# hpsim/OGL

Measured on AMD Instinct MI355X. Metric: cg_iters_per_sec, higher is better.
Workload: dtype f64

## Files before the change

### ogl_amd/csrc/kernels.hpp

```cpp
#pragma once
#include <hip/hip_runtime.h>

#include "common.hpp"

namespace ogl {

struct DevCriterion {
    double tolerance, rel_tol;
    int32_t min_iter, max_iter, frequency, export_res;
};

struct DevScalars {
    double rho, prev_rho, beta;
    double alpha, omega, gamma;
    double norm_factor;
    double init_res, res;
    double xbar;
    double sums[4];
    int32_t iter;
    int32_t stop;
    int32_t n_evals;
    int32_t stop_phase;
    int32_t stop_turn;
    int32_t comm_error;
// ... 63 lines not shown
    const int32_t *chunk_bptr = nullptr;
    const int32_t *boundary_rows = nullptr;
    const int32_t *entry_ptrs = nullptr;
    const int32_t *cols = nullptr;
    const double *vals = nullptr;
    const double *recv = nullptr;
    const unsigned long long *local_flag = nullptr;
    int32_t n_neigh = 0;
    uint32_t seq = 0;
    long long timeout_ticks = 0;
    DevScalars *s = nullptr;
};
void launch_spmv(hipStream_t st, const DevCsr &A, int mode, const double *x, const double *b,
                 double *y, const SpmvDots &dots, const DevScalars *gate, const HaloFused &hf = HaloFused{});

struct DevEll {
    int32_t n_rows = 0;
    int32_t width = 0;
    int64_t stride = 0;
    const int32_t *cols = nullptr;
    const double *vals = nullptr;
    bool stream = false;
};
void launch_spmv_ell(hipStream_t st, const DevEll &A, int mode, const double *x, const double *b,
                     double *y, const SpmvDots &dots, const DevScalars *gate, const HaloFused &hf = HaloFused{});
struct DevSell {
    int32_t n_rows = 0;
    const SellChunk *chunks = nullptr;
    const int32_t *dict = nullptr;
    const uint8_t *codes = nullptr;
    const double *vals = nullptr;
    const int32_t *spill_chunk_ptr = nullptr, *spill_rows = nullptr, *spill_ptrs = nullptr, *spill_cols = nullptr;
    const double *spill_vals = nullptr;
    bool stream = false;
    int32_t xcd_group = 0;
    const uint16_t *rmap = nullptr;
    const int32_t *block_order = nullptr;
    int32_t n_blocks = 0;
};
void launch_spmv_sell(hipStream_t st, const DevSell &A, int mode, const double *x, const double *b,
                      double *y, const SpmvDots &dots, const DevScalars *gate, const HaloFused &hf = HaloFused{});
struct DevSym {
    int32_t n_rows = 0;
    int32_t nd = 0;
    int32_t d[4] = {0, 0, 0, 0};
    const uint8_t *mask = nullptr;
    const double *planes = nullptr;
    bool stream = false;
    const int32_t *block_order = nullptr;
    int32_t n_blocks = 0;
};
void launch_spmv_sym(hipStream_t st, const DevSym &A, int mode, const double *x, const double *b, double *y,
                     const SpmvDots &dots, const DevScalars *gate, const HaloFused &hf = HaloFused{});
struct DevSymx {
    int32_t n_rows = 0;
    const SymxChunk *chunks = nullptr, *chunks_general = nullptr;
    int32_t n_blocks_general = 0;
    const uint8_t *mask = nullptr;
    const double *planes = nullptr;
    const int32_t *ex_rowptr = nullptr, *ex_cols = nullptr;
    const int32_t *ex_lrow = nullptr;
    const double *ex_vals = nullptr;
    bool stream = false;
    bool fast = false;
    int32_t xcd_group = 0;
    int32_t n_blocks = 0;
};
void launch_spmv_symx(hipStream_t st, const DevSymx &A, int mode, const double *x, const double *b, double *y,
                      const SpmvDots &dots, const DevScalars *gate, const HaloFused &hf = HaloFused{});
void launch_gather_coeffs_masked(hipStream_t st, int64_t n, const int32_t *map, const double *source,
                                 double *out);
void launch_gather_sell(hipStream_t st, int32_t n_chunks, const SellChunk *chunks, const int32_t *map,
                        const double *source, double *out);

void launch_spmv_non_local(hipStream_t st, const DevHalo &H, int mode, const double *recv,
                           double *y, const DevScalars *gate);
void launch_pack(hipStream_t st, const DevHalo &H, const double *x, double *send,
                 const DevScalars *gate);

void launch_gather_coeffs(hipStream_t st, int32_t nnz, const int32_t *ldu_mapping,
                          const double *source, double *coeffs);
void launch_jacobi_generate(hipStream_t st, const DevCsr &A, double *inv_diag);
void launch_jacobi_generate_pos(hipStream_t st, const DevCsr &A, const int32_t *diag_pos, double *inv_diag);
void launch_jacobi_generate_diag(hipStream_t st, int32_t n_rows, const double *diag, double *inv_diag);

struct DevBlockJacobi {
    int32_t n_rows = 0;
    int32_t n_blocks = 0;
    int32_t stride = 0;
    const int32_t *block_ptrs = nullptr;
    const int32_t *row_block = nullptr;
    double *blocks = nullptr;
    int32_t uniform = 0;
    const int32_t *rows = nullptr, *pos = nullptr;
    int32_t by_device_row = 0;
    int32_t perm_xcd_group = 0;
};
constexpr int MAX_JACOBI_BLOCK = 32;
void launch_bj_generate(hipStream_t st, const DevCsr &A, const DevBlockJacobi &J,
                        bool group_lanes = true);
void launch_bj_apply(hipStream_t st, const DevBlockJacobi &J, const double *in, double *out,
                     double *dot_part, const DevScalars *gate);
void launch_bj_apply_staged(hipStream_t st, const DevBlockJacobi &J, const double *in, double *out, double *dot_part,
                            const DevScalars *gate, double *tmp_in, double *tmp_out);

constexpr int ISAI_THREAD_ROW = 32;
// ... 336 lines not shown
```

### ogl_amd/csrc/kernels_krylov.hip

```cpp
#include "device_common.hpp"
#include "resident_cg_turn.hpp"

namespace ogl {

namespace {

__global__ __launch_bounds__(BLOCK) void k_scale(int n, double *__restrict__ v, double f)
{
    const int i = blockIdx.x * BLOCK + threadIdx.x;
    if (i < n) v[i] = v[i] * f;
}

__global__ __launch_bounds__(BLOCK) void k_fill_xbar(int n, double *__restrict__ v,
                                                     const DevScalars *s)
{
    const int i = blockIdx.x * BLOCK + threadIdx.x;
    if (i < n) v[i] = s->xbar;
}

enum PartialOp { P_SUM = 0, P_DOT = 1, P_NORM1 = 2 };
template <int OP>
__global__ __launch_bounds__(BLOCK) void k_partials(int n, int n_chunks,
                                                    const double *__restrict__ a,
                                                    const double *__restrict__ b,
// ... 238 lines not shown
        part_norm[chunk] = s1;
    }
    if (PUT) {
        __shared__ double ps[CHUNK_ROWS];
        __shared__ int last;
        halo_put_chunk(put, chunk, vz.x, vz.y, ps, &last);
    }
}


template <bool LEAD, int K>
__global__ __launch_bounds__(BLOCK) void k_cg_step1x_fin(int n, double *p, double *__restrict__ x,
                                                         const double *__restrict__ r,
                                                         const double *__restrict__ inv_diag,
                                                         const DevScalars *sin, DevScalars *sout,
                                                         const double *__restrict__ part_rho,
                                                         const double *__restrict__ part_norm, int n_part,
                                                         double *history, int first, LeadBox lead,
                                                         double *p_out, PRing ring)
{
    __shared__ double red[2 * FIN_WAVES];
    __shared__ double sh[4];
    __shared__ int sh_stop;
    __shared__ double lead_words[LEAD ? LEAD_BOX_WORDS / 2 : 1];
    __shared__ double lead_stage[LEAD ? LEAD_STAGE : 1];
    __shared__ int lead_timed_out;
    const uint32_t seq = LEAD ? sin->launch_seq : 0u;
    if (LEAD) lead_leaders<2>(lead, seq, part_rho, part_norm, nullptr, n_part, lead_stage);
    const int stopped = sin->stop;
    const double s_rho = sin->rho, s_beta = sin->beta, s_nf = sin->norm_factor, s_init = sin->init_res;
    const int phase = K > 0 ? ring.phase : 0;
    const bool defers = K > 0 && phase != 0;
    const unsigned s_pending = K > 0 && !first ? (unsigned)sin->defer_valid : 0u;
    constexpr int KQ = K > 0 ? K : 1;
    double s_t[KQ];
#pragma unroll
    for (int i = 1; i < KQ; ++i) s_t[i] = sin->t_ring[i];
    const int s_iter = sin->iter, s_evals = sin->n_evals;
    const CritVals crit = load_criterion(sin->crit);
    static_assert(sizeof(DevScalars) % 8 == 0, "copied as 8-byte words");
    if (blockIdx.x == 0 && threadIdx.x < sizeof(DevScalars) / 8)
        reinterpret_cast<unsigned long long *>(sout)[threadIdx.x] =
            reinterpret_cast<const unsigned long long *>(sin)[threadIdx.x];
    const RowPair rp = my_rows(blockIdx.x, n);
    double2 vp, vx, vz, vi, vq[KQ];
    vi.x = vi.y = 1.0;
    auto load_pending = [&](int upto) {
#pragma unroll
        for (int i = 1; i < KQ; ++i)
            if (i < upto && ((s_pending >> i) & 1u)) vq[i] = ld2(ring.b[i], rp);
    };
    const bool early = !LEAD || lead.early_loads != 0;
    const bool own_term = !first && s_beta != 0.0;
    if (early) {
        vp = ld2(p, rp);
        if (!defers) {
            vx = ld2_stream(x, rp);
            load_pending(KQ);
        }
        vz = ld2_stream(r, rp);
        if (inv_diag) vi = ld2_stream(inv_diag, rp);
    }
    auto update_x = [&](int upto) {
        bool any = own_term;
#pragma unroll
        for (int i = 1; i < KQ; ++i)
            if (i < upto && ((s_pending >> i) & 1u)) {
                vx.x += s_t[i] * vq[i].x;
                vx.y += s_t[i] * vq[i].y;
                any = true;
            }
        if (own_term) {
            const double t = s_rho / s_beta;
            vx.x += t * vp.x;
            vx.y += t * vp.y;
        }
        if (any) st2_stream(x, rp, vx);
    };
    double pv[2][FIN_VT];
    if (!LEAD) load_partials_as_finaliser<2>(part_rho, part_norm, n_part, pv);
    if (stopped) return;
    double v[2] = {0.0, 0.0};
    if (LEAD) {
        if (early && !defers) update_x(KQ);
        if (!lead_wait(lead, 4 * FIN_WAVES, seq, lead_words, &lead_timed_out)) {
            if (threadIdx.x == 0) sout->comm_error = sout->stop = 1;
            return;
        }
        if (!early) {
            vp = ld2(p, rp);
            if (!defers) {
                vx = ld2_stream(x, rp);
                load_pending(KQ);
            }
            vz = ld2_stream(r, rp);
            if (inv_diag) vi = ld2_stream(inv_diag, rp);
        }
        if (threadIdx.x == 0) {
            v[0] = lead_total(lead_words, 0);
            v[1] = lead_total(lead_words, 1);
        }
    } else {
        reduce_partials_as_finaliser<2>(pv, n_part, red, v);
    }
    if (threadIdx.x == 0) {
        const double prev_rho = s_rho, rho = v[0];
        const Verdict cv =
            criterion_verdict(crit, s_iter, s_evals, s_init, s_nf, v[1], blockIdx.x == 0 ? history : nullptr);
        const int stop = cv.stop;
        sh[0] = s_beta;
        sh[1] = prev_rho;
        sh[2] = rho;
        sh_stop = stop;
        if (blockIdx.x == 0) {
            sout->prev_rho = prev_rho;
            sout->rho = rho;
            sout->x_pending = 0;
            store_verdict(sout, cv);
            if (LEAD) sout->launch_seq = seq + 1;
            sout->defer_valid = (defers && !stop) ? (int)(s_pending | (own_term ? 1u << phase : 0u)) : 0;
            if (defers && own_term) sout->t_ring[phase] = s_rho / s_beta;
        }
    }
    __syncthreads();
    const double prev = sh[1], rho = sh[2];
    const int stop = sh_stop;
    if (!defers && !(LEAD && early)) update_x(KQ);
    if (defers && stop) {
        vx = ld2_stream(x, rp);
        load_pending(phase);
        update_x(phase);
    }
    if (stop) return;
    const double tmp = (prev == 0.0) ? 0.0 : rho / prev;
    if (inv_diag) {
        vz.x = vz.x * vi.x;
        vz.y = vz.y * vi.y;
    }
    vp.x = vz.x + tmp * vp.x;
    vp.y = vz.y + tmp * vp.y;
    st2(p_out, rp, vp);
}

template <bool LEAD, int CPW>
__global__ __launch_bounds__(BLOCK) void k_cg_step2r_fin(int n, double *__restrict__ r,
                                                         const double *__restrict__ q,
// ... 1238 lines not shown
```

### ogl_amd/csrc/kernels_spmv_sym.hip

```cpp
#include <algorithm>

#include "device_common.hpp"
#include "resident_cg_turn.hpp"

namespace ogl {

namespace {

struct SymOffsets {
    int d[SYM_MAX_OFFSETS];
};
SymOffsets sym_offsets(const DevSym &A, bool *fast)
{
    SymOffsets off;
    for (int j = 0; j < SYM_MAX_OFFSETS; ++j) off.d[j] = A.d[j];
    *fast = A.nd >= 2 && A.d[1] == 1;
    for (int j = 2; j < A.nd; ++j) *fast = *fast && (A.d[j] % 2 == 0);
    return off;
}
template <int MODE, int ND, bool FAST, bool STREAM>
__device__ __forceinline__ double2 sym_rows(int chunk, const RowPair &rp, int n_rows, const SymOffsets &off,
                                            const uint8_t *__restrict__ mask, const double *__restrict__ planes,
                                            const double *__restrict__ x, const double *__restrict__ b,
                                            double2 &xd_out)
// ... 72 lines not shown
        const double p = up[0].y * xd.y;
        acc.y = (MODE == SPMV_RESIDUAL) ? acc.y - p : acc.y + p;
    }
#pragma unroll
    for (int j = 1; j < ND; ++j) {
        if ((m0 >> (ND - 1 + j)) & 1u) {
            const double p = up[j].x * xu[j].x;
            acc.x = (MODE == SPMV_RESIDUAL) ? acc.x - p : acc.x + p;
        }
        if ((m1 >> (ND - 1 + j)) & 1u) {
            const double p = up[j].y * xu[j].y;
            acc.y = (MODE == SPMV_RESIDUAL) ? acc.y - p : acc.y + p;
        }
    }
    return acc;
}

template <int MODE, int NDOT, int ND, bool FAST, bool STREAM>
__global__ __launch_bounds__(BLOCK) void k_spmv_sym(int n_rows, int n_chunks, SymOffsets off,
                                                    const uint8_t *__restrict__ mask,
                                                    const double *__restrict__ planes,
                                                    const double *__restrict__ x, const double *__restrict__ b,
                                                    double *__restrict__ y, const double *__restrict__ w,
                                                    double *__restrict__ dot_partials,
                                                    double *__restrict__ dot2_partials, const DevScalars *gate,
                                                    const int *__restrict__ block_order, HaloFused hf)
{
    __shared__ double slot[N_WAVES];
    __shared__ double ys[CHUNK_ROWS];
    if (gate && gate->stop) return;
    const int chunk = block_order ? block_order[blockIdx.x] : xcd_chunk(blockIdx.x);
    if (chunk < 0 || chunk >= n_chunks) return;
    const RowPair rp = my_rows(chunk, n_rows);
    double2 xd;
    double2 acc = sym_rows<MODE, ND, FAST, STREAM>(chunk, rp, n_rows, off, mask, planes, x, b, xd);
    if (hf.chunk_bptr) halo_fused_add<MODE>(hf, chunk, acc.x, acc.y, ys);
    st2(y, rp, acc);
    if (NDOT >= 1) {
        const double2 vw = ld2(w, rp);
        double d = 0.0, d2 = 0.0;
        if (rp.n > 0) {
            d += vw.x * acc.x;
            d2 += acc.x * acc.x;
        }
        if (rp.n > 1) {
            d += vw.y * acc.y;
            d2 += acc.y * acc.y;
        }
        const double s = block_sum(d, slot);
        if (threadIdx.x == 0) dot_partials[chunk] = s;
        if (NDOT >= 2) {
            const double s2 = block_sum(d2, slot);
            if (threadIdx.x == 0) dot2_partials[chunk] = s2;
        }
    }
}

template <int ND>
struct TurnSymRegs {
    double2 vd[2], vl[2][ND], vu[2][ND], up[ND], lo[ND];
};
template <int ND, bool FAST, bool STREAM>
__device__ __forceinline__ void turn_sym_load(TurnSymRegs<ND> &R, int chunk, const RowPair &rp, int n_rows,
                                              const SymOffsets &off, const double *__restrict__ planes,
                                              const double *__restrict__ p_in, const double *__restrict__ z)
{
    const int row = rp.row;
    const double *src[2] = {p_in, z};
    const int last = n_rows - 1, last_pair = last & ~1;
#pragma unroll
    for (int a = 0; a < 2; ++a) {
        const double *__restrict__ v = src[a];
        R.vd[a] = ld2(v, rp);
#pragma unroll
        for (int j = 1; j < ND; ++j) {
            if (FAST && j >= 2) {
                R.vl[a][j] = *reinterpret_cast<const double2 *>(v + min(max(row - off.d[j], 0), last_pair));
                R.vu[a][j] = *reinterpret_cast<const double2 *>(v + min(row + off.d[j], last_pair));
            } else if (FAST) {
                R.vl[a][j].x = v[min(max(row - 1, 0), last)];
                R.vl[a][j].y = R.vd[a].x;
                R.vu[a][j].x = R.vd[a].y;
                R.vu[a][j].y = v[min(row + 2, last)];
            } else {
                R.vl[a][j].x = v[min(max(row - off.d[j], 0), last)];
                R.vl[a][j].y = v[min(max(row + 1 - off.d[j], 0), last)];
                R.vu[a][j].x = v[min(row + off.d[j], last)];
                R.vu[a][j].y = v[min(row + 1 + off.d[j], last)];
            }
        }
    }
    const double *own = planes + (long)chunk * (ND * CHUNK_ROWS) + threadIdx.x * ROWS_PER_THREAD;
#pragma unroll
    for (int j = 0; j < ND; ++j)
        R.up[j] = (STREAM && (j == 0 || (FAST && j == 1))) ? ld_pair_stream(own + (long)j * CHUNK_ROWS)
                                                           : *reinterpret_cast<const double2 *>(own + (long)j * CHUNK_ROWS);
#pragma unroll
    for (int j = 1; j < ND; ++j) {
        const int r0 = max(row - off.d[j], 0), r1 = max(row + 1 - off.d[j], 0);
        const long a0 = (long)(r0 >> 9) * (ND * CHUNK_ROWS) + (long)j * CHUNK_ROWS + (r0 & (CHUNK_ROWS - 1));
        const long a1 = (long)(r1 >> 9) * (ND * CHUNK_ROWS) + (long)j * CHUNK_ROWS + (r1 & (CHUNK_ROWS - 1));
        if (FAST && j >= 2) {
            R.lo[j] = *reinterpret_cast<const double2 *>(planes + a0);
        } else if (FAST) {
            if (STREAM) {
                const double prev = __shfl_up(R.up[1].y, 1, WAVE);
// ... 292 lines not shown
    double beta;
    if (!turn_await_beta(a, ts, lds, beta)) return;
    resident_cg_turn<R, L, K>(src, a, ts, lds, z, f, beta);
}

}

void launch_spmv_sym(hipStream_t st, const DevSym &A, int mode, const double *x, const double *b, double *y,
                     const SpmvDots &dots, const DevScalars *gate, const HaloFused &hf)
{
    if (A.n_rows == 0) return;
    const int nc = (int)n_chunks(A.n_rows);
    const dim3 grid(A.block_order ? A.n_blocks : xcd_grid(nc)), block(BLOCK);
    bool fast;
    const SymOffsets off = sym_offsets(A, &fast);
#define OGL_SYM_K(MODE, NDOT, ND, FAST, STREAM)                                                                          \
    hipLaunchKernelGGL((k_spmv_sym<MODE, NDOT, ND, FAST, STREAM>), grid, block, 0, st, A.n_rows, nc, off, A.mask, A.planes, \
                       x, b, y, dots.with, dots.part, dots.part_yy, gate, A.block_order, hf)
#define OGL_SYM_ND(MODE, NDOT, ND)                   \
    do {                                             \
        if (fast && A.stream)                        \
            OGL_SYM_K(MODE, NDOT, ND, true, true);   \
        else if (fast)                               \
            OGL_SYM_K(MODE, NDOT, ND, true, false);  \
        else if (A.stream)                           \
            OGL_SYM_K(MODE, NDOT, ND, false, true);  \
        else                                         \
            OGL_SYM_K(MODE, NDOT, ND, false, false); \
    } while (0)
#define OGL_SYM(MODE, NDOT)                    \
    do {                                       \
        if (A.nd == 2)                         \
            OGL_SYM_ND(MODE, NDOT, 2);         \
        else if (A.nd == 3)                    \
            OGL_SYM_ND(MODE, NDOT, 3);         \
        else                                   \
            OGL_SYM_ND(MODE, NDOT, 4);         \
    } while (0)
    static_assert(SYM_MAX_OFFSETS == 4, "instantiations above");
    if (mode == SPMV_RESIDUAL) {
        OGL_SYM(SPMV_RESIDUAL, 0);
    } else if (dots.part && dots.part_yy) {
        OGL_SYM(SPMV_PLAIN, 2);
    } else if (dots.part) {
        OGL_SYM(SPMV_PLAIN, 1);
    } else {
        OGL_SYM(SPMV_PLAIN, 0);
    }
#undef OGL_SYM
#undef OGL_SYM_ND
#undef OGL_SYM_K
}

void launch_cg_turn_sym(hipStream_t st, const DevSym &A, const double *p_in, double *p_out, double *x, const double *z,
                        double *q, double *part_beta, const DevScalars *sin, DevScalars *sout,
                        const double *part_rho, const double *part_norm, double *history, int first, const LeadBox &lead)
{
    if (A.n_rows == 0) return;
    const int nc = (int)n_chunks(A.n_rows);
    const dim3 grid(A.block_order ? A.n_blocks : xcd_grid(nc)), block(BLOCK);
    const bool led = lead.box && nc >= 3 * FIN_WAVES;
    bool fast;
    const SymOffsets off = sym_offsets(A, &fast);
#define OGL_TURN_K(ND, FAST)                                                                                                  \
    do {                                                                                                                      \
        if (led)                                                                                                              \
            hipLaunchKernelGGL((k_cg_turn_sym<ND, FAST, true>), grid, block, 0, st, A.n_rows, nc, off, A.mask, A.planes, p_in, \
                               p_out, x, z, q, part_beta, sin, sout, part_rho, part_norm, nc, history, first, A.block_order,  \
                               lead);                                                                                         \
        else                                                                                                                  \
            hipLaunchKernelGGL((k_cg_turn_sym<ND, FAST, false>), grid, block, 0, st, A.n_rows, nc, off, A.mask, A.planes,     \
                               p_in, p_out, x, z, q, part_beta, sin, sout, part_rho, part_norm, nc, history, first,           \
                               A.block_order, LeadBox{});                                                                     \
    } while (0)
#define OGL_TURN_ND(ND)              \
    do {                             \
        if (fast)                    \
            OGL_TURN_K(ND, true);    \
        else                         \
            OGL_TURN_K(ND, false);   \
    } while (0)
    if (A.nd == 2)
        OGL_TURN_ND(2);
    else if (A.nd == 3)
        OGL_TURN_ND(3);
    else
        OGL_TURN_ND(4);
#undef OGL_TURN_ND
#undef OGL_TURN_K
}

void launch_cg_turn_sym_big(hipStream_t st, const DevSym &A, const double *p_in, double *p_out, double *x,
                            const double *z, double *q, double *part_beta, const DevScalars *s,
                            const HaloFused &hf, const double *p_halo_in, double *p_halo_out)
{
    if (A.n_rows == 0) return;
    const int nc = (int)n_chunks(A.n_rows);
    const dim3 grid(A.block_order ? A.n_blocks : xcd_grid(nc)), block(BLOCK);
    bool fast;
    const SymOffsets off = sym_offsets(A, &fast);
#define OGL_TURN_K(ND, FAST, STREAM)                                                                                \
    do {                                                                                                            \
        if (hf.chunk_bptr)                                                                                          \
            hipLaunchKernelGGL((k_cg_turn_sym_big<ND, FAST, STREAM, true>), grid, block, 0, st, A.n_rows, nc, off,  \
                               A.mask, A.planes, p_in, p_out, x, z, q, part_beta, s, A.block_order, hf, p_halo_in,  \
                               p_halo_out);                                                                         \
// ... 108 lines not shown
```

### ogl_amd/csrc/solver.hpp

```cpp
#pragma once
#include <hip/hip_runtime.h>

#include <algorithm>
#include <map>
#include <memory>
#include <string>
#include <vector>

#include "comm.hpp"
#include "common.hpp"
#include "host_matrix.hpp"
#include "kernels.hpp"
#include "setup_kernels.hpp"
#include "spmv_layouts.hpp"

namespace ogl {

struct MgLevel {
    int32_t n = 0, nnz = 0, n_coarse = 0;
    int passes = 0;
    bool own = true;
    DevBuf<int32_t> row_ptrs, cols;
    DevBuf<double> vals, inv_d;
    DevBuf<int32_t> agg, agg_ptr, agg_rows;
// ... 394 lines not shown
    std::vector<int32_t> fac_seg_fwd, fac_seg_bwd;
    ogl::DevBuf<double> d_part0, d_part1, d_part2;
    int64_t band_order_rows = 0;
    bool source_diag_valid = false;
    int64_t csr_band_rows = 0;
    uint64_t csr_band_pat = 0;
    int csr_band(int64_t *band);
    ogl::DevBuf<int32_t> d_band_order;
    ogl::DevBuf<double> d_part3, d_part4, d_part5;
    ogl::DevBuf<ogl::DevScalars> d_scal;
    ogl::DevBuf<double> d_history;
    ogl::DevScalars *h_scal = nullptr;
    hipEvent_t poll_ev[2] = {nullptr, nullptr};
    unsigned long long *lead_box = nullptr;
    unsigned long long *held_z_box = nullptr;
    size_t held_z_words = 0;
    int held_z_census = 0, held_z_census_grid = 0;
    unsigned *held_q_heads = nullptr;
    hipEvent_t chk_ev[2] = {nullptr, nullptr};
    bool x_resident = false, b_resident = false;
    ogl::PrecondData own_precond;
    const ogl::PrecondData *precond_data = nullptr;
    const double *precond = nullptr;

    std::map<std::string, double> props;

    std::vector<double> history;
    double t_update_matrix_ms = 0;
    std::vector<hipEvent_t> prof_ev;

    ~ogl_solver();

    int set_matrix(const ogl_ldu_view &ldu);
    int solve(const double *source, double *psi, ogl_perf *perf);
    int apply_resident(ogl_perf *perf);
    int upload_vec(ogl::DevBuf<double> &dst, const double *src);
    int ensure_vectors();
    int init_preconditioner();
    int generate_preconditioner(ogl::PrecondData &P);
    int generate_jacobi(ogl::PrecondData &P);
    int generate_block_jacobi(ogl::PrecondData &P, bool through_perm);
    int generate_isai(ogl::PrecondData &P, bool caller_numbering);
    int generate_factor(ogl::PrecondData &P);
    int prepare_apply();
    void apply_factor(const double *in, double *out, const ogl::DevScalars *gate, double *dot_part);
    int check_factor_breakdown(int32_t word);
    void apply_preconditioner(const double *in, double *out, const ogl::DevScalars *gate,
                              double *dot_part = nullptr);
    int dist_spmv(int mode, const double *x, const double *b, double *y, const ogl::SpmvDots &dots,
                  const ogl::DevScalars *gate, bool prepacked = false);
    void spmv_on(ogl::SpmvLayout l, int mode, const double *x, const double *b, double *y, const ogl::SpmvDots &dots,
                 const ogl::DevScalars *gate, const ogl::HaloFused &hf = ogl::HaloFused{});
    int finalize(int phase, ogl::FinArgs &a);
    int run_cg(ogl_perf *perf);
    int run_bicgstab(ogl_perf *perf);
    int run_krylov(ogl_perf *perf);
    ogl::MixedPart mixed;
    int mixed_requested(bool *on);
    int mixed_storage(const ogl::DevCriterion &crit, double inner_rel_tol, int inner_max_iter);
    int mixed_overflow(const ogl::MixedScalars &m);
    void mixed_spmv(const float *x, float *y, double *part, const ogl::MixedScalars *gate);
    int run_mixed(ogl_perf *perf);
    int ortho_requested(int *method);
    int spmv_f32(const float *x, float *y);
    struct KrylovRun;
    int krylov_plan(KrylovRun &k);
    int krylov_prepare(KrylovRun &k);
    int krylov_loop(KrylovRun &k);
    int krylov_enqueue(KrylovRun &k, int count);
    int krylov_finish(KrylovRun &k, ogl_perf *perf);
    int gmres_restart(KrylovRun &k, const ogl::DevScalars *gate);
    int gmres_update_x(KrylovRun &k, int cols, const ogl::DevScalars *gate);
    int turn_gmres(KrylovRun &k, int enq, int pe);
    int time_ortho_kernels(KrylovRun &k);
    int turn_cg_generic(KrylovRun &k, int enq, int pe);
    int turn_cg_generic_led(KrylovRun &k, int enq, int pe);
    int turn_cg_two_launch(KrylovRun &k, int enq, int pe);
    int turn_cg_three_launch(KrylovRun &k, int enq, int pe);
    int turn_cg_held_z(KrylovRun &k, int enq, int pe);
    int turn_cg_held_q(KrylovRun &k, int enq, int pe);
    int plan_held_z(KrylovRun &k);
    int turn_cg_merged(KrylovRun &k, int enq, int pe);
    int turn_cg_five_launch(KrylovRun &k, int enq, int pe);
    int turn_bicg_folded(KrylovRun &k, int enq, int pe);
    int turn_bicg(KrylovRun &k, int enq, int pe);
    int time_spmv(int repeats, double *avg_ms);
    ogl::DevHalo halo() const;
    double prop(const std::string &key, double dflt) const;
    const ogl_solver *share_from = nullptr;
    const double *offdiag_upper = nullptr, *offdiag_lower = nullptr;
    uint64_t offdiag_sum = 0;
    bool offdiag_valid = false;
    const ogl_label *seen_lower_addr = nullptr, *seen_upper_addr = nullptr;
    ogl_label seen_faces = -1;
    struct SeenIface {
        const ogl_label *face_cells;
        ogl_label size, kind, neighb_proc, neighb_patch;
    };
    std::vector<SeenIface> seen_iface_cells;
    bool saw_addressing(const ogl_ldu_view &ldu) const;
    bool peer_safe_wait() const;
    double stream_above_bytes() const;
    double turn_extra_bytes() const;
    int32_t xcd_group() const;
    int32_t pat_xcd_group = 0;
};
// ... 1 lines not shown
```

### ogl_amd/csrc/solver_krylov.cpp

```cpp
#include "launch_key.hpp"
#include "solver_internal.hpp"

#include <algorithm>
#include <cmath>
#include <cstring>
#include <vector>

using namespace ogl;

HaloPutFused ogl_solver::begin_halo_put()
{
    HaloPutFused put;
    if (!(pat.non_local_nnz > 0 && peer_halo) || prop("haloFused", 1.0) == 0.0 || peer_safe_wait())
        return put;
    if (++halo_seq == 0) ++halo_seq;
    cur_halo = peer_halo_args(halo_seq);
    put.P = cur_halo;
    put.chunk_sptr = d_chunk_sptr.p;
    put.send_pos = d_send_pos.p;
    put.send_idxs = d_send_idxs.p;
    put.ticket = d_ticket.p;
    put.n_put_chunks = n_put_chunks;
    return put;
}
// ... 219 lines not shown
                       prop("fusedFinalizers", 1.0) != 0.0;
    const bool lead_any = !multi && !small && nc >= 3 * 16 && prop("leadFinalizers", 1.0) != 0.0;
    const bool lead_ok = lead_any && !bicg && !gmres;
    bool fused = k.fused = !bicg && !gmres && ((small && !generic) || lead_ok);
    k.lead = LeadBox{};
    k.s2 = s + 1;
    k.bicg_fold = bicg && (small || lead_any) && prop("bicgFold", 1.0) != 0.0;
    OGL_TRY(ortho_requested(&k.ortho));
    props["orthoMethodInUse"] = (double)k.ortho;
    k.gmres_fold = gmres && !k.ortho && (small || (lead_any && prop("gmresLead", 0.0) != 0.0)) && prop("gmresFold", 1.0) != 0.0;
    if (gmres)
        props["gmresLaunchesPerTurn"] =
            2.0 + (k.ortho ? 2.0 + 2.0 * k.ortho : k.gmres_fold ? 0.5 * (k.m - 1) + 3.0 : (double)(k.m - 1) + 4.0);
    k.slot_s[0] = s;
    k.slot_s[1] = k.s2;
    props["fusedFinalizersInUse"] = ((fused || k.bicg_fold || k.gmres_fold) && small) ? 1.0 : 0.0;
    bool merged = !bicg && !gmres && !generic && nc >= 1 && spmv_layout == SpmvLayout::Sym &&
                  ((fused && small) ? prop("fusedTurn", 1.0) != 0.0 : prop("fusedTurnBig", sym().stream ? 0.0 : 1.0) != 0.0);
    if (multi)
        merged = merged && peer_halo && prop("haloFused", 1.0) != 0.0 && prop("fusedTurnMulti", 1.0) != 0.0 &&
                 !peer_safe_wait();
    k.n_global = (double)n;
    if (multi) {
        const double mine[2] = {(double)n, merged ? 0.0 : 1.0};
        double got[2] = {0.0, 0.0};
        OGL_HIP_CHECK(hipMemcpyAsync(sums_ptr(s), mine, sizeof(mine), hipMemcpyHostToDevice, st));
        OGL_HIP_CHECK(hipStreamSynchronize(st));
        OGL_TRY(reg->allreduce(sums_ptr(s), 2));
        OGL_HIP_CHECK(hipMemcpyAsync(got, sums_ptr(s), sizeof(got), hipMemcpyDeviceToHost, st));
        OGL_HIP_CHECK(hipStreamSynchronize(st));
        k.n_global = got[0];
        merged = got[1] == 0.0;
    }
    if ((lead_ok && fused) || (lead_any && (k.bicg_fold || k.gmres_fold))) {
        if (!lead_box) {
            void *b = nullptr;
            OGL_HIP_CHECK(ledger::dev_malloc(&b, LEAD_REPLICAS * LEAD_REPLICA_STRIDE * sizeof(unsigned long long), true));
            lead_box = static_cast<unsigned long long *>(b);
        }
        OGL_HIP_CHECK(hipMemsetAsync(lead_box, 0, LEAD_REPLICAS * LEAD_REPLICA_STRIDE * sizeof(unsigned long long), st));
        k.lead.box = lead_box;
        k.lead.timeout_ticks = (long long)(prop("leadTimeoutS", 10.0) * 1e8);
        k.lead.early_loads = prop("leadEarlyLoads", 1.0) != 0.0 ? 1 : 0;
    }
    props["leadFinalizersInUse"] = k.lead.box ? 1.0 : 0.0;
    props["fusedFinalizersInUse"] = ((fused || k.bicg_fold || k.gmres_fold) && small) ? 1.0 : 0.0;
    k.merged = merged;
    k.fused2 = fused && merged;
    k.merged_halo = merged && multi && pat.non_local_nnz > 0;
    props["fusedTurnInUse"] = merged ? 1.0 : 0.0;
    return OGL_OK;
}

int ogl_solver::krylov_prepare(KrylovRun &k)
{
    hipStream_t st = k.st;
    const int n = k.n, nc = k.nc, m = k.m;
    DevScalars *s = k.s;
    const bool bicg = k.bicg, gmres = k.gmres, generic = k.generic, merged = k.merged;
    int ring_k = 0;
    if (k.lead.box != nullptr && k.fused && !k.fused2 && prop("deferX2", 1.0) != 0.0) {
        const double want = prop("deferX", 2.0);
        ring_k = want >= 8.0 ? 8 : want >= 4.0 ? 4 : want >= 2.0 ? 2 : 0;
    }
    props["deferXInUse"] = (double)ring_k;
    props["deferX2InUse"] = ring_k ? 1.0 : 0.0;
    if (merged || ring_k) OGL_TRY(d_p2.alloc((size_t)n + 2, st));
    for (int i = 2; i < ring_k; ++i) OGL_TRY(d_pring[i - 2].alloc((size_t)n + 2, st));
    if (merged && precond) OGL_TRY(d_z.alloc((size_t)n + 2, st));
    k.n_halo = (size_t)pat.non_local_nnz;
    if (k.merged_halo) {
        OGL_TRY(d_p_halo.alloc(2 * k.n_halo + 2, st));
        OGL_HIP_CHECK(hipMemsetAsync(d_p_halo.p, 0, d_p_halo.n * sizeof(double), st));
    }
    k.p0 = d_p.p;
    k.p1 = d_p2.p;
    k.ring.k = ring_k;
    for (int i = 0; i < ring_k; ++i) k.ring.b[i] = i == 0 ? d_p.p : i == 1 ? d_p2.p : d_pring[i - 2].p;
    k.ph = d_p_halo.p;
    k.z_kept = merged && precond ? d_z.p : nullptr;
    OGL_TRY(plan_held_z(k));

    k.is_final = cfg.rel_tol == 0.0;
    const int prev_iters = (int)prop(k.is_final ? "prevSolveIters_final" : "prevSolveIters", 1);
    const double prev_cost = prop("_prev_solve", 0.0);
    DevCriterion &crit = k.crit;
    crit.tolerance = cfg.tolerance;
    crit.rel_tol = cfg.rel_tol;
    crit.max_iter = bicg ? 2 * cfg.max_iter : cfg.max_iter;
    crit.export_res = cfg.export_res;
    ogl_host_adapt_criterion(&cfg, prev_iters, prev_cost, &crit.min_iter, &crit.frequency);
    if (crit.frequency < 1) return fail(OGL_ERR_INVALID, "evalFrequency must be >= 1");
    k.max_checks = std::max(crit.max_iter, crit.min_iter) + crit.frequency + 1;
    k.max_turns = bicg ? k.max_checks / 2 + 1 : k.max_checks;
    OGL_TRY(d_history.alloc((size_t)std::max(k.max_checks, crit.max_iter + std::max(1, cfg.norm_eval_limit) + 1) + 4, st));
    if (cfg.export_res)
        OGL_HIP_CHECK(hipMemsetAsync(d_history.p, 0, d_history.n * sizeof(double), st));
    if (k.bicg_fold) {
        OGL_TRY(d_part3.alloc((size_t)nc, st));
        OGL_TRY(d_part4.alloc((size_t)nc, st));
        OGL_TRY(d_part5.alloc((size_t)nc, st));
    }
    if (bicg) {
        const size_t nv = (size_t)n + 2;
        OGL_TRY(d_v.alloc(nv, st));
        OGL_TRY(d_s.alloc(nv, st));
        OGL_TRY(d_t.alloc(nv, st));
        OGL_TRY(d_rr.alloc(nv, st));
        if (precond || generic) {
            OGL_TRY(d_y.alloc(nv, st));
            OGL_TRY(d_z.alloc(nv, st));
        }
    } else if (gmres) {
        OGL_TRY(d_V.alloc((size_t)(m + 1) * (size_t)k.ldv, st));
        OGL_TRY(d_gm.alloc(gmres_state_len(m), st));
        OGL_HIP_CHECK(hipMemsetAsync(d_gm.p, 0, gmres_state_len(m) * sizeof(double), st));
        if (generic) OGL_TRY(d_z.alloc((size_t)n + 2, st));
        if (k.ortho) {
            OGL_TRY(d_gs_part.alloc((size_t)(m + 1) * (size_t)nc, st));
            OGL_TRY(d_gs_h.alloc((size_t)m + 1, st));
        }
    } else if (generic) {
        OGL_TRY(d_z.alloc((size_t)n + 2, st));
    }

    k.prof_stride = std::max(0, cfg.profile_kernels);
    k.prof_cap = k.prof_stride ? std::min((k.max_turns + k.prof_stride - 1) / k.prof_stride, 4096) : 0;
    while ((int)prof_ev.size() < 2 * k.prof_cap) {
        hipEvent_t e;
        OGL_HIP_CHECK(ev_create(&e));
        prof_ev.push_back(e);
    }
    for (int i = 0; i < 2; ++i) {
        if (!chk_ev[i]) OGL_HIP_CHECK(ev_create(&chk_ev[i]));
        k.ev_chk[i] = chk_ev[i];
    }

    k.t_start = now_ms();
    launch_reset_scalars(st, s, crit);

    FinArgs fa;
    launch_partials_sum(st, n, d_x.p, d_part0.p);
    fa = FinArgs{};
    fa.part[0] = d_part0.p;
    fa.n_part = nc;
    fa.n_sums = 1;
    fa.n_local = (double)n;
    fa.n_global = k.n_global;
    OGL_TRY(finalize(FIN_MEAN, fa));
    launch_fill_xbar(st, n, d_w.p, s);
    OGL_TRY(dist_spmv(SPMV_PLAIN, d_w.p, nullptr, d_q.p, SpmvDots{}, nullptr));
    OGL_TRY(dist_spmv(SPMV_RESIDUAL, d_x.p, d_b.p, d_r.p, SpmvDots{}, nullptr));
    launch_partials_normfactor(st, n, d_b.p, d_q.p, d_r.p, d_part0.p);
    fa = FinArgs{};
    fa.part[0] = d_part0.p;
    fa.n_part = nc;
    fa.n_sums = 1;
    OGL_TRY(finalize(FIN_NORMFACTOR, fa));

    OGL_HIP_CHECK(hipMemsetAsync(d_p.p, 0, (size_t)n * sizeof(double), st));
    k.fg = FinArgs{};
    k.fg.part[0] = d_part0.p;
    k.fg.part[1] = d_part1.p;
    k.fg.n_part = nc;
    k.fg.history = d_history.p;
    k.fg.gm = d_gm.p;
    k.fg.m = m;
    k.beta_ptr = reinterpret_cast<const double *>(reinterpret_cast<const char *>(s) + offsetof(DevScalars, beta));
    k.gm = d_gm.p;
    k.gm_y = d_gm.p + (size_t)(m + 1) * m + 2 * (size_t)m + (m + 1);
    if (gmres) {
        OGL_HIP_CHECK(hipEventRecord(k.ev_chk[0], st));
        OGL_TRY(gmres_restart(k, nullptr));
        OGL_HIP_CHECK(hipEventRecord(k.ev_chk[1], st));
    } else if (bicg) {
        OGL_HIP_CHECK(hipMemcpyAsync(d_rr.p, d_r.p, (size_t)n * sizeof(double),
                                     hipMemcpyDeviceToDevice, st));
        OGL_HIP_CHECK(hipMemsetAsync(d_v.p, 0, (size_t)n * sizeof(double), st));
        launch_cg_rho_norm(st, n, d_r.p, nullptr, d_part0.p, d_part1.p, s);
    } else {
        launch_cg_rho_norm(st, n, d_r.p, precond, d_part0.p, d_part1.p, s);
        if (k.z_kept) launch_mul(st, n, k.z_kept, d_r.p, precond, nullptr);
        if (generic) {
            apply_preconditioner(d_r.p, d_z.p, s, d_part0.p);
        }
    }
    k.chk = FinArgs{};
    k.chk.part[0] = d_part0.p;
    k.chk.part[1] = d_part1.p;
    k.chk.n_part = nc;
    k.chk.n_sums = 2;
    k.chk.history = d_history.p;
    if (!gmres && !k.folded()) {
        OGL_HIP_CHECK(hipEventRecord(k.ev_chk[0], st));
        OGL_TRY(finalize(FIN_CG_CHECK, k.chk));
        OGL_HIP_CHECK(hipEventRecord(k.ev_chk[1], st));
    }
    if (k.merged_halo) {
        if (++halo_seq == 0) ++halo_seq;
        cur_halo = peer_halo_args(halo_seq);
        launch_pack_put_signal(st, halo(), cur_halo, k.z_kept ? k.z_kept : d_r.p, s, d_ticket.p);
    }

    k.f1 = FinArgs{};
    k.f1.part[0] = d_part0.p;
    k.f1.n_part = nc;
    k.f1.n_sums = 1;
    k.f1.history = d_history.p;
    k.f2 = k.f1;
    k.f2.part[1] = d_part1.p;
    k.f2.n_sums = 2;

    k.y = (precond || generic) ? d_y.p : d_p.p;
    k.z = (precond || generic) ? d_z.p : d_s.p;
    k.enq = 0;
    return OGL_OK;
}

int ogl_solver::gmres_restart(KrylovRun &k, const DevScalars *gate)
{
    launch_cg_rho_norm(k.st, k.n, d_r.p, nullptr, d_part0.p, d_part1.p, gate);
    k.fg.n_sums = 2;
    k.fg.check_after = gate ? 0 : 1;
    OGL_TRY(finalize(FIN_GMRES_RESTART, k.fg));
    k.fg.check_after = 0;
    if (!k.gmres_scale_late()) launch_gmres_scale(k.st, k.n, d_V.p, d_r.p, k.beta_ptr, gate);
    return OGL_OK;
}

int ogl_solver::gmres_update_x(KrylovRun &k, int cols, const DevScalars *gate)
{
    if (cols <= 0) return OGL_OK;
    k.fg.n_sums = 0;
    k.fg.turn = cols;
// ... 716 lines not shown
```

### ogl_amd/csrc/solver_mixed.cpp

```cpp
#include "solver_internal.hpp"

#include <algorithm>
#include <climits>
#include <cmath>
#include <vector>

using namespace ogl;

namespace {

const char *solver_name(int kind)
{
    return kind == OGL_SOLVER_CG ? "GKOCG" : kind == OGL_SOLVER_BICGSTAB ? "GKOBiCGStab" : "GKOGMRES";
}

int32_t *word_of(MixedScalars *m, size_t offset) { return reinterpret_cast<int32_t *>(reinterpret_cast<char *>(m) + offset); }

}

int ogl_solver::mixed_requested(bool *on)
{
    *on = prop("mixedPrecision", 0.0) != 0.0;
    if (!*on) return OGL_OK;
    const double inner_rel_tol = prop("innerRelTol", 1e-4), inner_max_iter = prop("innerMaxIter", 1000.0);
// ... 40 lines not shown
        launch_mixed_spmv_csr(reg->stream, csr(false), fp32_dev.vals.p, x, y, part, gate);
}

int ogl_solver::mixed_overflow(const MixedScalars &m)
{
    if (m.bad_coef == INT_MAX && m.bad_invd == INT_MAX) return OGL_OK;
    fp32_dev.epoch = 0;
    const bool coef = m.bad_coef != INT_MAX;
    int64_t row = m.bad_invd;
    if (coef && fp32_dev.half) {
        const int64_t per_chunk = (int64_t)sym_dev.nd * CHUNK_ROWS;
        row = (m.bad_coef / per_chunk) * CHUNK_ROWS + m.bad_coef % CHUNK_ROWS;
    } else if (coef) {
        std::vector<int32_t> rp((size_t)pat.n_rows + 1);
        OGL_HIP_CHECK(hipMemcpy(rp.data(), d_row_ptrs.p, rp.size() * sizeof(int32_t), hipMemcpyDeviceToHost));
        row = (int64_t)(std::upper_bound(rp.begin(), rp.end(), m.bad_coef) - rp.begin()) - 1;
    }
    row = std::max<int64_t>(0, std::min<int64_t>(row, (int64_t)pat.n_rows - 1));
    if (pat.renumbered() && (size_t)row < pat.old_of.size()) row = pat.old_of[(size_t)row];
    return fail(OGL_ERR_INVALID, "mixedPrecision: %s of row %lld is finite in double precision and not in single precision",
                coef ? "a coefficient" : "the inverse diagonal", (long long)row);
}

int ogl_solver::run_mixed(ogl_perf *perf)
{
    hipStream_t st = reg->stream;
    const int n = pat.n_rows, nc = (int)n_chunks(n);
    DevScalars *s = d_scal.p;
    const bool is_final = cfg.rel_tol == 0.0;
    DevCriterion crit{};
    crit.tolerance = cfg.tolerance;
    crit.rel_tol = cfg.rel_tol;
    crit.min_iter = cfg.min_iter;
    crit.max_iter = cfg.max_iter;
    crit.frequency = 1;
    crit.export_res = cfg.export_res;
    const int inner_max_iter = (int)std::min(prop("innerMaxIter", 1000.0), 2147483647.0);
    OGL_TRY(mixed_storage(crit, prop("innerRelTol", 1e-4), inner_max_iter));
    MixedScalars *m = mixed.scal.p;
    const float *inv_d = nullptr;
    if (precond) {
        launch_mixed_refresh(st, n, nullptr, precond, mixed.inv_d.p, word_of(m, offsetof(MixedScalars, bad_invd)));
        inv_d = mixed.inv_d.p;
    }
    float *z = inv_d ? mixed.z.p : mixed.r.p;
    OGL_TRY(d_history.alloc((size_t)std::max(std::max(crit.max_iter, crit.min_iter) + 2,
                                             crit.max_iter + std::max(1, cfg.norm_eval_limit) + 1) + 4, st));
    if (cfg.export_res) OGL_HIP_CHECK(hipMemsetAsync(d_history.p, 0, d_history.n * sizeof(double), st));
    for (int i = 0; i < 2; ++i)
        if (!chk_ev[i]) OGL_HIP_CHECK(ev_create(&chk_ev[i]));

    const double t_start = now_ms();
    launch_reset_scalars(st, s, crit);
    launch_partials_sum(st, n, d_x.p, d_part0.p);
    FinArgs fa{};
    fa.part[0] = d_part0.p;
    fa.n_part = nc;
    fa.n_sums = 1;
    fa.n_local = fa.n_global = (double)n;
    OGL_TRY(finalize(FIN_MEAN, fa));
    launch_fill_xbar(st, n, d_w.p, s);
    OGL_TRY(dist_spmv(SPMV_PLAIN, d_w.p, nullptr, d_q.p, SpmvDots{}, nullptr));
    OGL_TRY(dist_spmv(SPMV_RESIDUAL, d_x.p, d_b.p, d_r.p, SpmvDots{}, nullptr));
    launch_partials_normfactor(st, n, d_b.p, d_q.p, d_r.p, d_part0.p);
    fa = FinArgs{};
    fa.part[0] = d_part0.p;
    fa.n_part = nc;
    fa.n_sums = 1;
    OGL_TRY(finalize(FIN_NORMFACTOR, fa));
    launch_partials_norm1(st, n, d_r.p, d_part2.p);

    auto poll_record = [&](int slot) -> int {
        OGL_HIP_CHECK(hipMemcpyAsync(&mixed.h_scal[slot], m, sizeof(MixedScalars), hipMemcpyDeviceToHost, st));
        OGL_HIP_CHECK(hipEventRecord(poll_ev[slot], st));
        return OGL_OK;
    };
    auto enqueue_turns = [&](int count) {
        for (int i = 0; i < count; ++i) {
            launch_mixed_step1(st, n, mixed.p.p, z, m);
            mixed_spmv(mixed.p.p, mixed.q.p, d_part2.p, m);
            launch_mixed_fin_pi(st, m, d_part2.p, nc);
            launch_mixed_step2(st, n, mixed.u.p, mixed.r.p, mixed.p.p, mixed.q.p, inv_d, mixed.z.p, d_part0.p, d_part1.p, m);
        }
    };
    const int batch = 16;
    int turns = 0, enqueued = 0;
    MixedScalars fin{};
    for (int k = 0;; ++k) {
        if (k == 0) OGL_HIP_CHECK(hipEventRecord(chk_ev[0], st));
        launch_mixed_head(st, m, s, d_part2.p, nc, d_history.p);
        if (k == 0) OGL_HIP_CHECK(hipEventRecord(chk_ev[1], st));
        launch_mixed_start(st, n, d_r.p, inv_d, mixed.r.p, z, mixed.u.p, d_part0.p, d_part1.p, m);
        const int cap = std::max(0, std::min(inner_max_iter, crit.max_iter - turns));
        int enq = 0;
        auto next_batch = [&]() {
            const int count = std::min(batch, cap - enq);
            enqueue_turns(count);
            enq += count;
            enqueued += count;
        };
        next_batch();
        OGL_TRY(poll_record(0));
        MixedScalars seen{};
        for (int j = 0;; ++j) {
            const bool more = enq < cap;
            if (more) {
                next_batch();
                OGL_TRY(poll_record((j + 1) & 1));
            }
            OGL_HIP_CHECK(hipEventSynchronize(poll_ev[j & 1]));
            seen = mixed.h_scal[j & 1];
            if (seen.outer_stop || seen.inner_stop) break;
            if (!more) return fail(OGL_ERR_STATE, "mixedPrecision: the inner solve did not stop within its budget");
        }
        if (seen.outer_stop) {
            fin = seen;
            break;
        }
        turns += seen.inner_turns;
        launch_mixed_add(st, n, d_x.p, mixed.u.p, m);
        OGL_TRY(dist_spmv(SPMV_RESIDUAL, d_x.p, d_b.p, d_r.p, SpmvDots{}, s));
        launch_partials_norm1(st, n, d_r.p, d_part2.p);
// ... 76 lines not shown
```

Before: 5044.

## Fuse CG prologue SpMVs, norm factor and rho into one symmetric kernel

Adds a fused prologue kernel for the symmetric stencil layout. It computes the residual r = b - Ax, the A*xbar term for the norm factor, and optionally the rho and norm partials in a single pass, replacing the fill_xbar, two SpMVs, the normfactor partials and the rho_norm launch. The first CG turn skips loading p and x when first is set, which allows the memset of p to be skipped on the fused path. This reduces one-time setup launches and memory traffic per solve, at the cost of extra template instantiations and a path that is restricted to single-rank runs with no halo.

```diff
diff --git a/ogl_amd/csrc/kernels.hpp b/ogl_amd/csrc/kernels.hpp
--- a/ogl_amd/csrc/kernels.hpp
+++ b/ogl_amd/csrc/kernels.hpp
@@ -139,6 +139,9 @@
 };
 void launch_spmv_sym(hipStream_t st, const DevSym &A, int mode, const double *x, const double *b, double *y,
                      const SpmvDots &dots, const DevScalars *gate, const HaloFused &hf = HaloFused{});
+void launch_prologue_sym(hipStream_t st, const DevSym &A, const double *x, const double *b, double *r,
+                         const double *inv_diag, double *part_nf, double *part_rho, double *part_norm,
+                         const DevScalars *s);
 struct DevSymx {
     int32_t n_rows = 0;
     const SymxChunk *chunks = nullptr, *chunks_general = nullptr;
diff --git a/ogl_amd/csrc/kernels_krylov.hip b/ogl_amd/csrc/kernels_krylov.hip
--- a/ogl_amd/csrc/kernels_krylov.hip
+++ b/ogl_amd/csrc/kernels_krylov.hip
@@ -314,11 +314,14 @@
     };
     const bool early = !LEAD || lead.early_loads != 0;
     const bool own_term = !first && s_beta != 0.0;
+    vp.x = vp.y = vx.x = vx.y = 0.0;
     if (early) {
-        vp = ld2(p, rp);
-        if (!defers) {
-            vx = ld2_stream(x, rp);
-            load_pending(KQ);
+        if (!first) {
+            vp = ld2(p, rp);
+            if (!defers) {
+                vx = ld2_stream(x, rp);
+                load_pending(KQ);
+            }
         }
         vz = ld2_stream(r, rp);
         if (inv_diag) vi = ld2_stream(inv_diag, rp);
@@ -350,10 +353,12 @@
             return;
         }
         if (!early) {
-            vp = ld2(p, rp);
-            if (!defers) {
-                vx = ld2_stream(x, rp);
-                load_pending(KQ);
+            if (!first) {
+                vp = ld2(p, rp);
+                if (!defers) {
+                    vx = ld2_stream(x, rp);
+                    load_pending(KQ);
+                }
             }
             vz = ld2_stream(r, rp);
             if (inv_diag) vi = ld2_stream(inv_diag, rp);
diff --git a/ogl_amd/csrc/kernels_spmv_sym.hip b/ogl_amd/csrc/kernels_spmv_sym.hip
--- a/ogl_amd/csrc/kernels_spmv_sym.hip
+++ b/ogl_amd/csrc/kernels_spmv_sym.hip
@@ -148,6 +148,157 @@
         if (NDOT >= 2) {
             const double s2 = block_sum(d2, slot);
             if (threadIdx.x == 0) dot2_partials[chunk] = s2;
+        }
+    }
+}
+
+template <int ND, bool FAST, bool STREAM>
+__device__ __forceinline__ void sym_rows_two(int chunk, const RowPair &rp, int n_rows, const SymOffsets &off,
+                                             const uint8_t *__restrict__ mask, const double *__restrict__ planes,
+                                             const double *__restrict__ x, double xbar, const double2 &vb, double2 &res,
+                                             double2 &axb)
+{
+    const int t = threadIdx.x;
+    const int row = rp.row;
+    const unsigned mm = *reinterpret_cast<const unsigned short *>(mask + row);
+    const unsigned m0 = mm & 0xffu, m1 = mm >> 8;
+    double2 up[ND];
+    const double *own = planes + (long)chunk * (ND * CHUNK_ROWS) + t * ROWS_PER_THREAD;
+#pragma unroll
+    for (int j = 0; j < ND; ++j)
+        up[j] = (STREAM && (j == 0 || (FAST && j == 1))) ? ld_pair_stream(own + (long)j * CHUNK_ROWS)
+                                                         : *reinterpret_cast<const double2 *>(own + (long)j * CHUNK_ROWS);
+    const double2 xd = ld2(x, rp);
+    const int last = n_rows - 1, last_pair = last & ~1;
+    double2 lo[ND];
+#pragma unroll
+    for (int j = 1; j < ND; ++j) {
+        const int r0 = max(row - off.d[j], 0), r1 = max(row + 1 - off.d[j], 0);
+        const long a0 = (long)(r0 >> 9) * (ND * CHUNK_ROWS) + (long)j * CHUNK_ROWS + (r0 & (CHUNK_ROWS - 1));
+        const long a1 = (long)(r1 >> 9) * (ND * CHUNK_ROWS) + (long)j * CHUNK_ROWS + (r1 & (CHUNK_ROWS - 1));
+        if (FAST && j >= 2) {
+            lo[j] = *reinterpret_cast<const double2 *>(planes + a0);
+        } else if (FAST) {
+            if (STREAM) {
+                lo[j].x = __shfl_up(up[1].y, 1, WAVE);
+                if ((t & (WAVE - 1)) == 0) lo[j].x = planes[a0];
+            } else {
+                lo[j].x = planes[a0];
+            }
+            lo[j].y = up[1].x;
+        } else {
+            lo[j].x = planes[a0];
+            lo[j].y = planes[a1];
+        }
+    }
+    static_assert(CHUNK_ROWS == 512, "row >> 9 above");
+    double2 xl[ND], xu[ND];
+#pragma unroll
+    for (int j = 1; j < ND; ++j) {
+        if (FAST && j >= 2) {
+            xl[j] = *reinterpret_cast<const double2 *>(x + min(max(row - off.d[j], 0), last_pair));
+            xu[j] = *reinterpret_cast<const double2 *>(x + min(row + off.d[j], last_pair));
+        } else if (FAST) {
+            xl[j].x = x[min(max(row - 1, 0), last)];
+            xl[j].y = xd.x;
+            xu[j].x = xd.y;
+            xu[j].y = x[min(row + 2, last)];
+        } else {
+            xl[j].x = x[min(max(row - off.d[j], 0), last)];
+            xl[j].y = x[min(max(row + 1 - off.d[j], 0), last)];
+            xu[j].x = x[min(row + off.d[j], last)];
+            xu[j].y = x[min(row + 1 + off.d[j], last)];
+        }
+    }
+    res = vb;
+    axb.x = axb.y = 0.0;
+#pragma unroll
+    for (int j = ND - 1; j >= 1; --j) {
+        if ((m0 >> (ND - 1 - j)) & 1u) {
+            res.x = res.x - lo[j].x * xl[j].x;
+            axb.x = axb.x + lo[j].x * xbar;
+        }
+        if ((m1 >> (ND - 1 - j)) & 1u) {
+            res.y = res.y - lo[j].y * xl[j].y;
+            axb.y = axb.y + lo[j].y * xbar;
+        }
+    }
+    if ((m0 >> (ND - 1)) & 1u) {
+        res.x = res.x - up[0].x * xd.x;
+        axb.x = axb.x + up[0].x * xbar;
+    }
+    if ((m1 >> (ND - 1)) & 1u) {
+        res.y = res.y - up[0].y * xd.y;
+        axb.y = axb.y + up[0].y * xbar;
+    }
+#pragma unroll
+    for (int j = 1; j < ND; ++j) {
+        if ((m0 >> (ND - 1 + j)) & 1u) {
+            res.x = res.x - up[j].x * xu[j].x;
+            axb.x = axb.x + up[j].x * xbar;
+        }
+        if ((m1 >> (ND - 1 + j)) & 1u) {
+            res.y = res.y - up[j].y * xu[j].y;
+            axb.y = axb.y + up[j].y * xbar;
+        }
+    }
+}
+
+template <bool RHO, int ND, bool FAST, bool STREAM>
+__global__ __launch_bounds__(BLOCK) void k_prologue_sym(int n_rows, int n_chunks, SymOffsets off,
+                                                        const uint8_t *__restrict__ mask,
+                                                        const double *__restrict__ planes,
+                                                        const double *__restrict__ x, const double *__restrict__ b,
+                                                        double *__restrict__ r, const double *__restrict__ inv_diag,
+                                                        double *__restrict__ part_nf, double *__restrict__ part_rho,
+                                                        double *__restrict__ part_norm, const DevScalars *s,
+                                                        const int *__restrict__ block_order)
+{
+    __shared__ double slot[N_WAVES];
+    const int chunk = block_order ? block_order[blockIdx.x] : xcd_chunk(blockIdx.x);
+    if (chunk < 0 || chunk >= n_chunks) return;
+    const RowPair rp = my_rows(chunk, n_rows);
+    const double xbar = s->xbar;
+    const double2 vb = ld2(b, rp);
+    double2 vi;
+    vi.x = vi.y = 1.0;
+    if (RHO && inv_diag) vi = ld2(inv_diag, rp);
+    double2 vr, vw;
+    sym_rows_two<ND, FAST, STREAM>(chunk, rp, n_rows, off, mask, planes, x, xbar, vb, vr, vw);
+    st2(r, rp, vr);
+    double d = 0.0;
+    if (rp.n > 0) {
+        const double t = vb.x - 1.0 * vw.x;
+        const double p2 = fabs(t);
+        d += fabs(fabs(t - 1.0 * vr.x) + 1.0 * p2);
+    }
+    if (rp.n > 1) {
+        const double t = vb.y - 1.0 * vw.y;
+        const double p2 = fabs(t);
+        d += fabs(fabs(t - 1.0 * vr.y) + 1.0 * p2);
+    }
+    const double sd = block_sum(d, slot);
+    if (threadIdx.x == 0) part_nf[chunk] = sd;
+    if (RHO) {
+        double2 vz = vr;
+        if (inv_diag) {
+            vz.x = vr.x * vi.x;
+            vz.y = vr.y * vi.y;
+        }
+        double e = 0.0, a = 0.0;
+        if (rp.n > 0) {
+            e += vr.x * vz.x;
+            a += fabs(vr.x);
+        }
+        if (rp.n > 1) {
+            e += vr.y * vz.y;
+            a += fabs(vr.y);
+        }
+        const double s0 = block_sum(e, slot);
+        const double s1 = block_sum(a, slot);
+        if (threadIdx.x == 0) {
+            part_rho[chunk] = s0;
+            part_norm[chunk] = s1;
         }
     }
 }
@@ -546,6 +697,48 @@
 #undef OGL_SYM_K
 }
 
+void launch_prologue_sym(hipStream_t st, const DevSym &A, const double *x, const double *b, double *r,
+                         const double *inv_diag, double *part_nf, double *part_rho, double *part_norm,
+                         const DevScalars *s)
+{
+    if (A.n_rows == 0) return;
+    const int nc = (int)n_chunks(A.n_rows);
+    const dim3 grid(A.block_order ? A.n_blocks : xcd_grid(nc)), block(BLOCK);
+    bool fast;
+    const SymOffsets off = sym_offsets(A, &fast);
+#define OGL_PRO_K(RHO, ND, FAST, STREAM)                                                                                   \
+    hipLaunchKernelGGL((k_prologue_sym<RHO, ND, FAST, STREAM>), grid, block, 0, st, A.n_rows, nc, off, A.mask, A.planes, x, \
+                       b, r, inv_diag, part_nf, part_rho, part_norm, s, A.block_order)
+#define OGL_PRO_ND(RHO, ND)                   \
+    do {                                      \
+        if (fast && A.stream)                 \
+            OGL_PRO_K(RHO, ND, true, true);   \
+        else if (fast)                        \
+            OGL_PRO_K(RHO, ND, true, false);  \
+        else if (A.stream)                    \
+            OGL_PRO_K(RHO, ND, false, true);  \
+        else                                  \
+            OGL_PRO_K(RHO, ND, false, false); \
+    } while (0)
+#define OGL_PRO(RHO)                \
+    do {                            \
+        if (A.nd == 2)              \
+            OGL_PRO_ND(RHO, 2);     \
+        else if (A.nd == 3)         \
+            OGL_PRO_ND(RHO, 3);     \
+        else                        \
+            OGL_PRO_ND(RHO, 4);     \
+    } while (0)
+    static_assert(SYM_MAX_OFFSETS == 4, "instantiations above");
+    if (part_rho)
+        OGL_PRO(true);
+    else
+        OGL_PRO(false);
+#undef OGL_PRO
+#undef OGL_PRO_ND
+#undef OGL_PRO_K
+}
+
 void launch_cg_turn_sym(hipStream_t st, const DevSym &A, const double *p_in, double *p_out, double *x, const double *z,
                         double *q, double *part_beta, const DevScalars *sin, DevScalars *sout,
                         const double *part_rho, const double *part_norm, double *history, int first, const LeadBox &lead)
diff --git a/ogl_amd/csrc/solver.hpp b/ogl_amd/csrc/solver.hpp
--- a/ogl_amd/csrc/solver.hpp
+++ b/ogl_amd/csrc/solver.hpp
@@ -470,6 +470,7 @@
     void spmv_on(ogl::SpmvLayout l, int mode, const double *x, const double *b, double *y, const ogl::SpmvDots &dots,
                  const ogl::DevScalars *gate, const ogl::HaloFused &hf = ogl::HaloFused{});
     int finalize(int phase, ogl::FinArgs &a);
+    int solve_prologue(double n_global, bool want_rho, bool *rho_done);
     int run_cg(ogl_perf *perf);
     int run_bicgstab(ogl_perf *perf);
     int run_krylov(ogl_perf *perf);
diff --git a/ogl_amd/csrc/solver_krylov.cpp b/ogl_amd/csrc/solver_krylov.cpp
--- a/ogl_amd/csrc/solver_krylov.cpp
+++ b/ogl_amd/csrc/solver_krylov.cpp
@@ -295,6 +295,44 @@
     return OGL_OK;
 }
 
+int ogl_solver::solve_prologue(double n_global, bool want_rho, bool *rho_done)
+{
+    hipStream_t st = reg->stream;
+    const int n = pat.n_rows, nc = (int)n_chunks(n);
+    DevScalars *s = d_scal.p;
+    *rho_done = false;
+    const bool one_pass = prop("fusedPrologue", 1.0) != 0.0 && !reg->comm->multi() && pat.non_local_nnz == 0 &&
+                          spmv_layout == SpmvLayout::Sym && nc >= 1;
+    props["fusedPrologueInUse"] = one_pass ? 1.0 : 0.0;
+    FinArgs fa;
+    launch_partials_sum(st, n, d_x.p, d_part0.p);
+    fa = FinArgs{};
+    fa.part[0] = d_part0.p;
+    fa.n_part = nc;
+    fa.n_sums = 1;
+    fa.n_local = (double)n;
+    fa.n_global = n_global;
+    OGL_TRY(finalize(FIN_MEAN, fa));
+    double *part_nf = d_part0.p;
+    if (one_pass) {
+        part_nf = d_part2.p;
+        launch_prologue_sym(st, sym(), d_x.p, d_b.p, d_r.p, precond, part_nf, want_rho ? d_part0.p : nullptr,
+                            want_rho ? d_part1.p : nullptr, s);
+        *rho_done = want_rho;
+    } else {
+        launch_fill_xbar(st, n, d_w.p, s);
+        OGL_TRY(dist_spmv(SPMV_PLAIN, d_w.p, nullptr, d_q.p, SpmvDots{}, nullptr));
+        OGL_TRY(dist_spmv(SPMV_RESIDUAL, d_x.p, d_b.p, d_r.p, SpmvDots{}, nullptr));
+        launch_partials_normfactor(st, n, d_b.p, d_q.p, d_r.p, part_nf);
+    }
+    fa = FinArgs{};
+    fa.part[0] = part_nf;
+    fa.n_part = nc;
+    fa.n_sums = 1;
+    OGL_TRY(finalize(FIN_NORMFACTOR, fa));
+    return OGL_OK;
+}
+
 int ogl_solver::krylov_prepare(KrylovRun &k)
 {
     hipStream_t st = k.st;
@@ -381,27 +419,11 @@
 
     k.t_start = now_ms();
     launch_reset_scalars(st, s, crit);
-
-    FinArgs fa;
-    launch_partials_sum(st, n, d_x.p, d_part0.p);
-    fa = FinArgs{};
-    fa.part[0] = d_part0.p;
-    fa.n_part = nc;
-    fa.n_sums = 1;
-    fa.n_local = (double)n;
-    fa.n_global = k.n_global;
-    OGL_TRY(finalize(FIN_MEAN, fa));
-    launch_fill_xbar(st, n, d_w.p, s);
-    OGL_TRY(dist_spmv(SPMV_PLAIN, d_w.p, nullptr, d_q.p, SpmvDots{}, nullptr));
-    OGL_TRY(dist_spmv(SPMV_RESIDUAL, d_x.p, d_b.p, d_r.p, SpmvDots{}, nullptr));
-    launch_partials_normfactor(st, n, d_b.p, d_q.p, d_r.p, d_part0.p);
-    fa = FinArgs{};
-    fa.part[0] = d_part0.p;
-    fa.n_part = nc;
-    fa.n_sums = 1;
-    OGL_TRY(finalize(FIN_NORMFACTOR, fa));
-
-    OGL_HIP_CHECK(hipMemsetAsync(d_p.p, 0, (size_t)n * sizeof(double), st));
+    bool rho_done = false;
+    OGL_TRY(solve_prologue(k.n_global, !bicg && !gmres && !generic, &rho_done));
+
+    if (!(k.fused && !k.fused2 && prop("fusedPrologue", 1.0) != 0.0))
+        OGL_HIP_CHECK(hipMemsetAsync(d_p.p, 0, (size_t)n * sizeof(double), st));
     k.fg = FinArgs{};
     k.fg.part[0] = d_part0.p;
     k.fg.part[1] = d_part1.p;
@@ -422,7 +444,7 @@
         OGL_HIP_CHECK(hipMemsetAsync(d_v.p, 0, (size_t)n * sizeof(double), st));
         launch_cg_rho_norm(st, n, d_r.p, nullptr, d_part0.p, d_part1.p, s);
     } else {
-        launch_cg_rho_norm(st, n, d_r.p, precond, d_part0.p, d_part1.p, s);
+        if (!rho_done) launch_cg_rho_norm(st, n, d_r.p, precond, d_part0.p, d_part1.p, s);
         if (k.z_kept) launch_mul(st, n, k.z_kept, d_r.p, precond, nullptr);
         if (generic) {
             apply_preconditioner(d_r.p, d_z.p, s, d_part0.p);
diff --git a/ogl_amd/csrc/solver_mixed.cpp b/ogl_amd/csrc/solver_mixed.cpp
--- a/ogl_amd/csrc/solver_mixed.cpp
+++ b/ogl_amd/csrc/solver_mixed.cpp
@@ -116,22 +116,8 @@
 
     const double t_start = now_ms();
     launch_reset_scalars(st, s, crit);
-    launch_partials_sum(st, n, d_x.p, d_part0.p);
-    FinArgs fa{};
-    fa.part[0] = d_part0.p;
-    fa.n_part = nc;
-    fa.n_sums = 1;
-    fa.n_local = fa.n_global = (double)n;
-    OGL_TRY(finalize(FIN_MEAN, fa));
-    launch_fill_xbar(st, n, d_w.p, s);
-    OGL_TRY(dist_spmv(SPMV_PLAIN, d_w.p, nullptr, d_q.p, SpmvDots{}, nullptr));
-    OGL_TRY(dist_spmv(SPMV_RESIDUAL, d_x.p, d_b.p, d_r.p, SpmvDots{}, nullptr));
-    launch_partials_normfactor(st, n, d_b.p, d_q.p, d_r.p, d_part0.p);
-    fa = FinArgs{};
-    fa.part[0] = d_part0.p;
-    fa.n_part = nc;
-    fa.n_sums = 1;
-    OGL_TRY(finalize(FIN_NORMFACTOR, fa));
+    bool rho_done = false;
+    OGL_TRY(solve_prologue((double)n, false, &rho_done));
     launch_partials_norm1(st, n, d_r.p, d_part2.p);
 
     auto poll_record = [&](int slot) -> int {
```

After: 5099, median of 6. No clear change (+1.1%).
